# nabeelscicom/DistilCodec_nabeel

Measured on AMD Instinct MI355X. Metric: 24 kHz samples/s encode+decode at 1/8 GPU; code-index bit-exact vs CPU, higher is better.
Workload: dtype f32

## Files before the change

### distilcodec_nabeel_amd/csrc/dcx_conv_h3.hip

```cpp
#include "dcx_conv_common.h"
#include "dcx_conv_launch.h"
#include "dcx_conv_pingpong.h"
#include "dcx_w3_layout.h"

namespace dcx {

DCX_DIAG_FILE(h3)

typedef _Float16 f16x8 __attribute__((ext_vector_type(8)));

template <int BM, int BN>
__device__ __forceinline__ bool ragged_tile_done(const ConvParams& p, const ConvParams& pr, int wg, int b, int ph) {
  int q0, co0;
  tile_origin<BM, BN>(p, wg, q0, co0);
  if (!tile_dead(p, pr, b, q0)) return false;
  epilogue_dead<BM, BN, 512>(p, pr, q0, co0, b, ph);
  return true;
}

template <int BN, int HALO, bool RAG = false>
__device__ __forceinline__ void x3dq_tile(const ConvParams& p, const ConvParams& pr, const int wg, const int b, const int ph) {
  constexpr int BM = 32768 / BN, WN = BN / 64, WM = 8 / WN;
  constexpr int NA = HALO ? 2 : 3;
  constexpr int WR = BM / WM, WC = BN / WN, TM = WR / 16, TN = WC / 16;
  constexpr int AR = BM + HALO;
  constexpr int A_G = AR / 16, B_G = BN / 16;
  constexpr int A_PW = A_G / 4, B_PW = B_G / 4;
  constexpr int ABUF = AR * 128, BBUF = BN * 128;
  constexpr int LDS_B = NA * ABUF + 3 * BBUF;
  static_assert(WR == 64 && WC == 64 && A_G % 4 == 0 && B_G % 4 == 0 && AR % 64 == 0, "tile shape");
  static_assert(LDS_B <= 160 * 1024, "LDS");
  __shared__ __attribute__((aligned(16))) unsigned short lds[LDS_B / 2];

  if constexpr (RAG)
    if (ragged_tile_done<BM, BN>(p, pr, wg, b, ph)) return;
  const TileGeo g = tile_geo<BM, BN, WN>(p, wg, ph, p.Cin / 32);
  const int lane = g.lane, group = g.group, gw = g.gw, wm = g.wm, wn = g.wn, q0 = g.q0, co0 = g.co0;
  const int nchunks = g.nchunks, taps = g.taps, nsteps = g.nsteps, lo_rel = g.lo_rel, row0 = g.row0;
  const int arow = p.ldx * 4;
  const __amdgpu_buffer_rsrc_t rx = x_desc<4, HALO>(p, b, row0, BM);
  const int rbase = HALO ? row0 : 0;
  const __amdgpu_buffer_rsrc_t rw = __builtin_amdgcn_make_buffer_rsrc(
      (void*)(p.w3 + w3_step(taps, p.Cin, p.Cout, ph, 0, 0)), 0, taps * nchunks * p.Cout * 128, 0x00020000);

  int a_off[A_PW], b_off[B_PW];
#pragma unroll
  for (int i = 0; i < A_PW; ++i) {
    const int u = (group * A_G + i * 4 + gw) * 64;
    const int pc = u / AR, row = u - pc * AR + lane;
    a_off[i] = (rbase + row) * arow + (pc & 3) * 32 + (pc >> 2) * 16;
  }
#pragma unroll
  for (int i = 0; i < B_PW; ++i) {
    b_off[i] = w3_wide_lane(co0, lane) + w3_wide_piece(BN, group * B_G + i * 4 + gw);
  }
  unsigned short* const a_dst = lds + (group * A_G + gw) * 512;
  unsigned short* const b_dst = lds + NA * ABUF / 2 + (group * B_G + gw) * 512;
  [[maybe_unused]] bool in_loop = false;
  auto dma_step = [&](int c, int m, int slot) {
#ifdef DCX_X3_NODMA
    if (in_loop) return 0;
#endif
    int n = B_PW;
    if (m == 0) {
#pragma unroll
      for (int i = 0; i < A_PW; ++i)
        dma16(rx, a_dst + (HALO ? (c & 1) : slot) * (ABUF / 2) + i * 2048, a_off[i] + c * 128, 0);
      n += A_PW;
    }
    const int soff = w3_step_bytes(nchunks, p.Cout, m, c);
#pragma unroll
    for (int i = 0; i < B_PW; ++i) dma16(rw, b_dst + slot * (BBUF / 2) + i * 2048, b_off[i], soff);
    return n;
  };

  const int l15 = lane & 15, kg = lane >> 4;
  const int pah = kg * AR * 16, pal = (4 + kg) * AR * 16;
  const int pbh = kg * BN * 16, pbl = (4 + kg) * BN * 16;
  const char* const ldsb = reinterpret_cast<const char*>(lds);
  const int bcol = NA * ABUF + (wn * WC + l15) * 16;
  s16x8 aq[TM][2], bq[TN][2];
  auto readF = [&](int c, int m, int slot) {
    const char* a = ldsb + (HALO ? (c & 1) : slot) * ABUF + (wm * WR + m * p.in_step - lo_rel + l15) * 16;
    const char* bb = ldsb + bcol + slot * BBUF;
#pragma unroll
    for (int j = 0; j < TN; ++j) {
      bq[j][0] = *reinterpret_cast<const s16x8*>(bb + j * 256 + pbh);
      bq[j][1] = *reinterpret_cast<const s16x8*>(bb + j * 256 + pbl);
    }
#pragma unroll
    for (int i = 0; i < TM; ++i) {
      aq[i][0] = *reinterpret_cast<const s16x8*>(a + i * 256 + pah);
      aq[i][1] = *reinterpret_cast<const s16x8*>(a + i * 256 + pal);
    }
  };
  f32x4 acc[TM][TN];
  zero_acc(acc);
  auto mfma = [&]() {
    __builtin_amdgcn_s_setprio(1);
#pragma unroll
    for (int k = 0; k < 3; ++k) {
      const int sa = k == 1 ? 1 : 0, sb = k == 0 ? 1 : 0;
#pragma unroll
      for (int i = 0; i < TM; ++i)
#pragma unroll
        for (int j = 0; j < TN; ++j)
          acc[i][j] = __builtin_amdgcn_mfma_f32_16x16x32_f16(__builtin_bit_cast(f16x8, aq[i][sa]),
                                                             __builtin_bit_cast(f16x8, bq[j][sb]), acc[i][j], 0, 0, 0);
    }
    __builtin_amdgcn_s_setprio(0);
  };

  const StepPos l3 = pingpong3_prologue(nsteps, taps, dma_step);
  const EpiPre epre = epi_range_pre<HALO == 0 ? 3 : 0>(p, pr, b);
  const float unscale = __builtin_bit_cast(float, __builtin_amdgcn_readfirstlane(__builtin_bit_cast(int,
      __builtin_ldexpf(1.0f, -(p.w3_shift + (pr.x_ash ? pr.x_ash[b] : pr.x_ash_c))))));
  pingpong3_drain();
  in_loop = true;
  pingpong3_loop<true>(group, nsteps, taps, l3, dma_step, readF, mfma);
#pragma unroll
  for (int i = 0; i < TM; ++i)
#pragma unroll
    for (int j = 0; j < TN; ++j) acc[i][j] *= unscale;
  epilogue_lds<BM, BN, WM, WN, LDS_B / 4, 512, HALO == 0 ? 3 : 0, RAG>(p, pr, acc, q0, co0, b, ph, reinterpret_cast<float*>(lds), &epre);
}

template <int BN, int HALO, bool RAG = false>
__global__ void __launch_bounds__(512, 2) conv_gemm_x3dq(const ConvParams p) {
  int wg, b, ph;
  flat_tile(((p.Lq + 32768 / BN - 1) / (32768 / BN)) * (p.Cout / BN), p.batch, wg, b, ph);
  x3dq_tile<BN, HALO, RAG>(p, p, wg, b, ph);
}

template <int BN, bool RAG = false>
__global__ void __launch_bounds__(512, 2) conv_gemm_x3dq_group(const ConvGroup g) {
  ConvParams p;
  int local, b;
  const ConvParams& pr = group_member(g, p, local, b);
  x3dq_tile<BN, 64, RAG>(p, pr, local, b, 0);
}

template <int HALO, bool SPLIT, int BN = 256, bool RAG = false>
__device__ __forceinline__ void x3dw_tile(const ConvParams& p, const ConvParams& pr, const int wg, const int b, const int ph) {
  constexpr int BM = BN == 256 ? 256 : 384, WN = BN / 128, WM = 8 / WN;
  constexpr int WR = BM / WM, WC = 128, TM = WR / 16, TN = WC / 16;
  constexpr int AR = BM + HALO;
  constexpr int A_N = AR / 8, B_N = BN / 8;
  constexpr int A_PW = A_N / 4;
  constexpr int ABUF = AR * 128, BBUF = BN * 128;
  constexpr int NA = 2;
  constexpr int LDS_B = NA * ABUF + 2 * BBUF;
  static_assert(A_N % 4 == 0 && B_N % 4 == 0 && AR % 64 == 0, "tile shape");
  static_assert(LDS_B + 16 <= 160 * 1024, "LDS");
  __shared__ __attribute__((aligned(16))) unsigned short lds[LDS_B / 2 + 8];
  unsigned int* const rd_cnt = reinterpret_cast<unsigned int*>(lds + LDS_B / 2);

  const int tid = threadIdx.x, lane = tid & 63;
  [[maybe_unused]] const int wave = tid >> 6;
  const int group = __builtin_amdgcn_readfirstlane(tid >> 8);
  const int gw = __builtin_amdgcn_readfirstlane((tid >> 6) & 3);
  const int wm = wave / WN, wn = wave % WN;
  const int ntiles = p.Cout / BN;
  const int mt = wg / ntiles, nt = wg - mt * ntiles;
  const int q0 = mt * BM, co0 = nt * BN;
  if (RAG && tile_dead(p, pr, b, q0)) {
    epilogue_dead<BM, BN, 512>(p, pr, q0, co0, b, ph);
    return;
  }
  const int nchunks = p.Cin / 32;
  const int taps = p.taps;
  const int nsteps = nchunks * taps;
  const int lo_rel = p.in_step < 0 ? (taps - 1) * p.in_step : 0;
  const int row0 = q0 + p.in_base[ph] + lo_rel;
  const int arow = p.ldx * 4;
  const __amdgpu_buffer_rsrc_t rx = x_desc<4, HALO>(p, b, row0, BM);
  const int rbase = HALO ? row0 : 0;
  const __amdgpu_buffer_rsrc_t rw = __builtin_amdgcn_make_buffer_rsrc(
      (void*)(p.w3 + w3_step(taps, p.Cin, p.Cout, ph, 0, 0)), 0, taps * nchunks * p.Cout * 128, 0x00020000);

  const int a_lane = (rbase + lane) * arow;
  const int b_lane = w3_wide_lane(co0, lane);
  [[maybe_unused]] bool in_loop = false;
  auto dmaA1 = [&](int c, int slot, int i) {
#ifdef DCX_X3_NODMA
    if (in_loop) return;
#endif
    const int k = i * 4 + gw;
    const int u = k * 64, pc = u / AR, row = u - pc * AR;
    const int abuf = HALO ? (c & 1) : slot;
    dma16(rx, lds + abuf * (ABUF / 2) + k * 512, a_lane + row * arow + (pc & 3) * 32 + (pc >> 2) * 16 + c * 128, 0);
  };
#ifndef DCX_X3W_BG0_DIV
#define DCX_X3W_BG0_DIV 2
#endif
  constexpr int B_G0 = !SPLIT ? B_N : HALO ? B_N / DCX_X3W_BG0_DIV : 0;
  constexpr int B_W0 = B_G0 / 4, B_W1 = (B_N - B_G0) / 4;
  auto dmaB1 = [&](int c, int m, int slot, int i) {
#ifdef DCX_X3_NODMA
    if (in_loop) return;
#endif
    const int k = (group ? B_G0 : 0) + i * 4 + gw;
    dma16(rw, lds + NA * ABUF / 2 + slot * (BBUF / 2) + k * 512, b_lane, w3_step_bytes(nchunks, p.Cout, m, c) + w3_wide_piece(BN, k));
  };
  auto dma_step = [&](int c, int m, int slot) {
    if (m == 0) {
#pragma unroll
      for (int i = 0; i < A_PW; ++i) dmaA1(c, slot, i);
    }
#pragma unroll
    for (int i = 0; i < B_W0; ++i) dmaB1(c, m, slot, i);
  };
  auto dma_step1 = [&](int c, int m, int slot) {
#pragma unroll
    for (int i = 0; i < B_W1; ++i) dmaB1(c, m, slot, i);
  };

  const int l15 = lane & 15, kg = lane >> 4;
  const char* const ldsb = reinterpret_cast<const char*>(lds);
  const char* const a_rd = ldsb + kg * AR * 16 + (wm * WR + l15) * 16;
  const char* const b_rd = ldsb + NA * ABUF + kg * BN * 16 + (wn * WC + l15) * 16;
  s16x8 aq[TM][2], bq[TN][2];
  auto readF = [&](int c, int m, int slot) {
    const char* a = a_rd + ((HALO ? (c & 1) : slot) * ABUF + (m * p.in_step - lo_rel) * 16);
    const char* bb = b_rd + slot * BBUF;
#pragma unroll
    for (int j = 0; j < TN; ++j) {
      bq[j][0] = *reinterpret_cast<const s16x8*>(bb + j * 256);
      bq[j][1] = *reinterpret_cast<const s16x8*>(bb + j * 256 + 4 * BN * 16);
    }
#pragma unroll
    for (int i = 0; i < TM; ++i) {
      aq[i][0] = *reinterpret_cast<const s16x8*>(a + i * 256);
      aq[i][1] = *reinterpret_cast<const s16x8*>(a + i * 256 + 4 * AR * 16);
    }
  };
  f32x4 acc[TM][TN];
  zero_acc(acc);
  auto mfma = [&]() {
    __builtin_amdgcn_s_setprio(1);
#pragma unroll
    for (int k = 0; k < 3; ++k) {
      const int sa = k == 1 ? 1 : 0, sb = k == 0 ? 1 : 0;
#pragma unroll
      for (int i = 0; i < TM; ++i) {
#pragma unroll
        for (int j = 0; j < TN; ++j)
          acc[i][j] = __builtin_amdgcn_mfma_f32_16x16x32_f16(__builtin_bit_cast(f16x8, aq[i][sa]),
                                                             __builtin_bit_cast(f16x8, bq[j][sb]), acc[i][j], 0, 0, 0);
      }
    }
    __builtin_amdgcn_s_setprio(0);
  };

  int cl = 0, ml = 0;
  if (SPLIT && tid == 0) *rd_cnt = 0u;
  for (int t = 0; t < 2 && t < nsteps; ++t) {
    if (group == 0) dma_step(cl, ml, t);
    else if (SPLIT) dma_step1(cl, ml, t);
    step_adv(cl, ml, taps);
  }
  const EpiPre epre = epi_range_pre<HALO == 0 ? 3 : 0>(p, pr, b);
  const float unscale = __builtin_bit_cast(float, __builtin_amdgcn_readfirstlane(__builtin_bit_cast(int,
      __builtin_ldexpf(1.0f, -(p.w3_shift + (pr.x_ash ? pr.x_ash[b] : pr.x_ash_c))))));
  asm volatile("s_waitcnt vmcnt(0)" ::: "memory");
  seg_barrier();
  in_loop = true;
#ifdef DCX_SEG_DIAG
  unsigned long long sd[6] = {};
#endif
  int cr = 0, mr = 0;
  if (group == 0) {
    readF(0, 0, 0);
    if (SPLIT) {
      asm volatile("s_waitcnt lgkmcnt(0)" ::: "memory");
      if (lane == 0) __hip_atomic_fetch_add(rd_cnt, 1u, __ATOMIC_RELAXED, __HIP_MEMORY_SCOPE_WORKGROUP);
    }
    step_adv(cr, mr, taps);
    for (int s = 0; s < nsteps; ++s) {
      DCX_SEGT(ta);
      mfma();
      asm volatile("s_waitcnt vmcnt(0)" ::: "memory");
      DCX_SEGT(tb);
      seg_barrier();
      DCX_SEGT(tc);
      if (s + 2 < nsteps) {
        dma_step(cl, ml, s & 1);
        step_adv(cl, ml, taps);
      }
      DCX_SEGT(tr);
      if (s + 1 < nsteps) readF(cr, mr, (s + 1) & 1);
      DCX_SEGT(tq);
      DCX_SEGT(td);
      seg_barrier();
      DCX_SEGT(te);
#ifdef DCX_SEG_DIAG
      sd[0] += tb - ta; sd[1] += tc - tb; sd[2] += td - tc; sd[3] += te - td; sd[4] += tr - tc; sd[5] += tq - tr;
#endif
      step_adv(cr, mr, taps);
    }
  } else {
    for (int s = 0; s < nsteps; ++s) {
      DCX_SEGT(ta);
      readF(cr, mr, s & 1);
      if (SPLIT) {
        int n = 0;
        if (s + 2 < nsteps) {
          asm volatile("s_waitcnt lgkmcnt(0)" ::: "memory");
          if (lane == 0) __hip_atomic_fetch_add(rd_cnt, 1u, __ATOMIC_RELAXED, __HIP_MEMORY_SCOPE_WORKGROUP);
          const unsigned int want = 4u * (unsigned)(s + 2);
          while (__hip_atomic_load(rd_cnt, __ATOMIC_RELAXED, __HIP_MEMORY_SCOPE_WORKGROUP) < want) {
          }
          dma_step1(cl, ml, s & 1);
          step_adv(cl, ml, taps);
          n = B_W1;
        }
        wait_dma(n);
      }
      DCX_SEGT(tb);
      seg_barrier();
      DCX_SEGT(tc);
      mfma();
      DCX_SEGT(td);
      seg_barrier();
      DCX_SEGT(te);
#ifdef DCX_SEG_DIAG
      sd[2] += tb - ta; sd[3] += tc - tb; sd[0] += td - tc; sd[1] += te - td; sd[5] += tb - ta;
#endif
      step_adv(cr, mr, taps);
    }
  }
#ifdef DCX_SEG_DIAG
  if ((threadIdx.x & 255) == 0) {
#pragma unroll
    for (int i = 0; i < 6; ++i) atomicAdd(&g_seg_diag[group * 6 + i], sd[i]);
    if (group == 0) atomicAdd(&g_seg_diag[12], (unsigned long long)nsteps);
  }
  if (lane == 0) {
#pragma unroll
    for (int i = 0; i < 6; ++i) atomicAdd(&g_seg_diag8[wave * 6 + i], sd[i]);
    if (wave == 0) atomicAdd(&g_seg_diag8[48], (unsigned long long)nsteps);
  }
#endif
  asm volatile("s_waitcnt vmcnt(0)" ::: "memory");
#pragma unroll
  for (int i = 0; i < TM; ++i)
#pragma unroll
    for (int j = 0; j < TN; ++j) acc[i][j] *= unscale;
  epilogue_lds<BM, BN, WM, WN, LDS_B / 4, 512, HALO == 0 ? 3 : 0, RAG>(p, pr, acc, q0, co0, b, ph, reinterpret_cast<float*>(lds), &epre);
}

template <int HALO, bool SPLIT, int BN = 256, bool RAG = false>
__global__ void __launch_bounds__(512, 2) conv_gemm_x3dw(const ConvParams p) {
  constexpr int BM = BN == 256 ? 256 : 384;
  int wg, b, ph;
  flat_tile(((p.Lq + BM - 1) / BM) * (p.Cout / BN), p.batch, wg, b, ph);
  x3dw_tile<HALO, SPLIT, BN, RAG>(p, p, wg, b, ph);
}

template <bool SPLIT, int BN = 256, bool RAG = false>
__global__ void __launch_bounds__(512, 2) conv_gemm_x3dw_group(const ConvGroup g) {
  ConvParams p;
  int local, b;
  const ConvParams& pr = group_member(g, p, local, b);
  x3dw_tile<64, SPLIT, BN, RAG>(p, pr, local, b, 0);
}

bool x3dq_ok(const ConvParams& p, int bn, bool wide) {
  const int span = (p.taps - 1) * (p.in_step < 0 ? -p.in_step : p.in_step);
  if (!p.x6 || !p.w3 || p.x_layout != LAYOUT_H2 || p.Cin % 32 || p.Cout % bn || p.ksplit > 1) return false;
  const long long arow = (long long)p.ldx * 4;
  if ((long long)p.taps * p.Cin * p.Cout * 4 >= (1LL << 31)) return false;
  if (p.taps == 1) {
    for (int i = 0; i < kMaxPhases; ++i)
      if (p.in_base[i] < 0) return false;
    return 256LL * arow < (1LL << 31);
  }
  return p.taps >= (wide ? 2 : 3) && span > 0 && span <= 64 && (long long)(p.Lin + 1024) * arow < (1LL << 31);
}
int x3dq_bn(const ConvParams& p) {
  const int k = p.kn ? p.kn->h3_bn : 0;
  if (p.Cout % 256) return (k == 128 && p.taps >= 3) || p.taps < 2 ? 128 : 384;
  if (p.taps == 2) return 512;
  return k == 128 ? 128 : k == 256 ? 256 : 512;
}

template <int BN>
hipError_t launch_x3dq(const ConvParams& p, int batch, int phases, hipStream_t s, const char** kname) {
  constexpr int BM = 32768 / BN;
  if (p.taps == 1) {
    if (p.clip_len) return hipErrorNotSupported;
    if (kname) *kname = BN == 256 ? "conv_gemm_x3dm<128,256>" : "conv_gemm_x3dm<256,128>";
    return launch_flat<BM, BN>(conv_gemm_x3dq<BN, 0>, p, batch, phases, 512, s);
  }
  if (kname) *kname = BN == 256 ? "conv_gemm_x3dq<128,256,halo>" : "conv_gemm_x3dq<256,128,halo>";
  if (p.clip_len) return launch_flat<BM, BN>(conv_gemm_x3dq<BN, 64, true>, p, batch, phases, 512, s);
  return launch_flat<BM, BN>(conv_gemm_x3dq<BN, 64>, p, batch, phases, 512, s);
}

template hipError_t launch_x3dq<256>(const ConvParams&, int, int, hipStream_t, const char**);
template hipError_t launch_x3dq<128>(const ConvParams&, int, int, hipStream_t, const char**);

hipError_t launch_x3dw(const ConvParams& p, int bsel, int batch, int phases, hipStream_t s, const char** kname) {
  const bool sp = knobs(p).h3_split;
  if (p.clip_len) {
    if (p.taps == 1) return hipErrorNotSupported;
    if (bsel == 384) {
      if (kname) *kname = "conv_gemm_x3dw<384,128,halo>";
      return sp ? launch_flat<384, 128>(conv_gemm_x3dw<64, true, 128, true>, p, batch, phases, 512, s)
                : launch_flat<384, 128>(conv_gemm_x3dw<64, false, 128, true>, p, batch, phases, 512, s);
    }
    if (kname) *kname = "conv_gemm_x3dw<256,256,halo>";
    return sp ? launch_flat<256, 256>(conv_gemm_x3dw<64, true, 256, true>, p, batch, phases, 512, s)
              : launch_flat<256, 256>(conv_gemm_x3dw<64, false, 256, true>, p, batch, phases, 512, s);
  }
  if (bsel == 384) {
    if (kname) *kname = "conv_gemm_x3dw<384,128,halo>";
    return sp ? launch_flat<384, 128>(conv_gemm_x3dw<64, true, 128>, p, batch, phases, 512, s)
              : launch_flat<384, 128>(conv_gemm_x3dw<64, false, 128>, p, batch, phases, 512, s);
  }
  if (p.taps == 1) {
    if (kname) *kname = "conv_gemm_x3dw<256,256>";
    return sp ? launch_flat<256, 256>(conv_gemm_x3dw<0, true>, p, batch, phases, 512, s)
              : launch_flat<256, 256>(conv_gemm_x3dw<0, false>, p, batch, phases, 512, s);
  }
  if (kname) *kname = "conv_gemm_x3dw<256,256,halo>";
  return sp ? launch_flat<256, 256>(conv_gemm_x3dw<64, true>, p, batch, phases, 512, s)
            : launch_flat<256, 256>(conv_gemm_x3dw<64, false>, p, batch, phases, 512, s);
}

hipError_t launch_h3_group(const ConvGroup& g, int bsel, bool split, unsigned blocks, hipStream_t s, const char** kname) {
  if (g.p[0].clip_len) {
    if (bsel == 384) {
      if (kname) *kname = "conv_gemm_x3dw_group<384,128,halo>";
      if (split) hipLaunchKernelGGL((conv_gemm_x3dw_group<true, 128, true>), dim3(blocks), dim3(512), 0, s, g);
      else hipLaunchKernelGGL((conv_gemm_x3dw_group<false, 128, true>), dim3(blocks), dim3(512), 0, s, g);
    } else if (bsel == 512) {
      if (kname) *kname = "conv_gemm_x3dw_group<256,256,halo>";
      if (split) hipLaunchKernelGGL((conv_gemm_x3dw_group<true, 256, true>), dim3(blocks), dim3(512), 0, s, g);
      else hipLaunchKernelGGL((conv_gemm_x3dw_group<false, 256, true>), dim3(blocks), dim3(512), 0, s, g);
    } else if (bsel == 256) {
      if (kname) *kname = "conv_gemm_x3dq_group<128,256,halo>";
      hipLaunchKernelGGL((conv_gemm_x3dq_group<256, true>), dim3(blocks), dim3(512), 0, s, g);
    } else {
      if (kname) *kname = "conv_gemm_x3dq_group<256,128,halo>";
      hipLaunchKernelGGL((conv_gemm_x3dq_group<128, true>), dim3(blocks), dim3(512), 0, s, g);
    }
    return hipGetLastError();
  }
  if (bsel == 384) {
    if (kname) *kname = "conv_gemm_x3dw_group<384,128,halo>";
    if (split) hipLaunchKernelGGL((conv_gemm_x3dw_group<true, 128>), dim3(blocks), dim3(512), 0, s, g);
    else hipLaunchKernelGGL((conv_gemm_x3dw_group<false, 128>), dim3(blocks), dim3(512), 0, s, g);
  } else if (bsel == 512) {
    if (kname) *kname = "conv_gemm_x3dw_group<256,256,halo>";
    if (split) hipLaunchKernelGGL(conv_gemm_x3dw_group<true>, dim3(blocks), dim3(512), 0, s, g);
    else hipLaunchKernelGGL(conv_gemm_x3dw_group<false>, dim3(blocks), dim3(512), 0, s, g);
  } else if (bsel == 256) {
    if (kname) *kname = "conv_gemm_x3dq_group<128,256,halo>";
    hipLaunchKernelGGL((conv_gemm_x3dq_group<256>), dim3(blocks), dim3(512), 0, s, g);
  } else {
    if (kname) *kname = "conv_gemm_x3dq_group<256,128,halo>";
    hipLaunchKernelGGL((conv_gemm_x3dq_group<128>), dim3(blocks), dim3(512), 0, s, g);
  }
  return hipGetLastError();
}

}
```

Baseline: 49.09 million.

## Use row-blocked XOR-swizzled LDS layout for A tiles in x3dw kernel

Replaces the column-plane LDS layout of the activation tile in the x3dw conv GEMM with a row-major 8-row block layout where each 128-byte row holds all k-pieces, XOR-swizzled by row bits. The DMA lanes now load 8 rows by 8 pieces per instruction, and the fragment reads use an XOR on the address to pick the second half-plane, which removes the per-instruction divide and aims to cut LDS bank conflicts and improve global coalescing. The new layout applies to every variant except the plain halo, non-split, BN=256, non-ragged, non-grouped case, which keeps the old path. It relies on the swizzle staying conflict-free when the rows are shifted by the halo offset.

```diff
diff --git a/distilcodec_nabeel_amd/csrc/dcx_a3_layout.h b/distilcodec_nabeel_amd/csrc/dcx_a3_layout.h
--- /dev/null
+++ b/distilcodec_nabeel_amd/csrc/dcx_a3_layout.h
@@ -0,0 +1,25 @@
+#pragma once
+
+#if defined(__HIPCC__) || defined(__CUDACC__)
+#define DCX_A3_HD __host__ __device__
+#else
+#define DCX_A3_HD
+#endif
+
+namespace dcx {
+
+constexpr int kA3BlockRows = 8;
+constexpr int kA3PlaneXor = 64;
+
+DCX_A3_HD constexpr int a3_swz(int row, int q) { return q ^ (row & 6); }
+DCX_A3_HD constexpr int a3_image(int row, int q) { return row * 128 + a3_swz(row, q) * 16; }
+
+DCX_A3_HD constexpr int a3_lane_row(int lane) { return lane >> 3; }
+DCX_A3_HD constexpr int a3_lane_piece(int lane) { return a3_swz(lane >> 3, lane & 7); }
+DCX_A3_HD constexpr int a3_piece_src(int q) { return (q & 3) * 32 + (q >> 2) * 16; }
+DCX_A3_HD constexpr int a3_src_lane(int rbase, int arow, int lane) {
+  return (rbase + a3_lane_row(lane)) * arow + a3_piece_src(a3_lane_piece(lane));
+}
+DCX_A3_HD constexpr int a3_src_inst(int arow, int k, int c) { return k * kA3BlockRows * arow + c * 128; }
+
+}
diff --git a/distilcodec_nabeel_amd/csrc/dcx_conv_h3.hip b/distilcodec_nabeel_amd/csrc/dcx_conv_h3.hip
--- a/distilcodec_nabeel_amd/csrc/dcx_conv_h3.hip
+++ b/distilcodec_nabeel_amd/csrc/dcx_conv_h3.hip
@@ -1,6 +1,7 @@
 #include "dcx_conv_common.h"
 #include "dcx_conv_launch.h"
 #include "dcx_conv_pingpong.h"
+#include "dcx_a3_layout.h"
 #include "dcx_w3_layout.h"
 
 namespace dcx {
@@ -140,7 +141,7 @@
   x3dq_tile<BN, 64, RAG>(p, pr, local, b, 0);
 }
 
-template <int HALO, bool SPLIT, int BN = 256, bool RAG = false>
+template <int HALO, bool SPLIT, int BN = 256, bool RAG = false, bool GROUPED = false>
 __device__ __forceinline__ void x3dw_tile(const ConvParams& p, const ConvParams& pr, const int wg, const int b, const int ph) {
   constexpr int BM = BN == 256 ? 256 : 384, WN = BN / 128, WM = 8 / WN;
   constexpr int WR = BM / WM, WC = 128, TM = WR / 16, TN = WC / 16;
@@ -178,7 +179,8 @@
   const __amdgpu_buffer_rsrc_t rw = __builtin_amdgcn_make_buffer_rsrc(
       (void*)(p.w3 + w3_step(taps, p.Cin, p.Cout, ph, 0, 0)), 0, taps * nchunks * p.Cout * 128, 0x00020000);
 
-  const int a_lane = (rbase + lane) * arow;
+  constexpr bool ROWS = !(HALO && !SPLIT && BN == 256 && !RAG && !GROUPED);
+  const int a_lane = ROWS ? a3_src_lane(rbase, arow, lane) : (rbase + lane) * arow;
   const int b_lane = w3_wide_lane(co0, lane);
   [[maybe_unused]] bool in_loop = false;
   auto dmaA1 = [&](int c, int slot, int i) {
@@ -186,9 +188,13 @@
     if (in_loop) return;
 #endif
     const int k = i * 4 + gw;
-    const int u = k * 64, pc = u / AR, row = u - pc * AR;
     const int abuf = HALO ? (c & 1) : slot;
-    dma16(rx, lds + abuf * (ABUF / 2) + k * 512, a_lane + row * arow + (pc & 3) * 32 + (pc >> 2) * 16 + c * 128, 0);
+    if constexpr (ROWS) {
+      dma16(rx, lds + abuf * (ABUF / 2) + k * 512, a_lane + a3_src_inst(arow, k, c), 0);
+    } else {
+      const int u = k * 64, pc = u / AR, row = u - pc * AR;
+      dma16(rx, lds + abuf * (ABUF / 2) + k * 512, a_lane + row * arow + (pc & 3) * 32 + (pc >> 2) * 16 + c * 128, 0);
+    }
   };
 #ifndef DCX_X3W_BG0_DIV
 #define DCX_X3W_BG0_DIV 2
@@ -217,11 +223,15 @@
 
   const int l15 = lane & 15, kg = lane >> 4;
   const char* const ldsb = reinterpret_cast<const char*>(lds);
-  const char* const a_rd = ldsb + kg * AR * 16 + (wm * WR + l15) * 16;
+  const int a_row = wm * WR + l15;
+  static_assert(WR % kA3BlockRows == 0 && a3_image(16, 0) == 2048, "row blocks as immediates");
   const char* const b_rd = ldsb + NA * ABUF + kg * BN * 16 + (wn * WC + l15) * 16;
   s16x8 aq[TM][2], bq[TN][2];
   auto readF = [&](int c, int m, int slot) {
-    const char* a = a_rd + ((HALO ? (c & 1) : slot) * ABUF + (m * p.in_step - lo_rel) * 16);
+    const int a_r = a_row + (HALO ? m * p.in_step - lo_rel : 0);
+    const int ah = (HALO ? (c & 1) : slot) * ABUF + (ROWS ? a3_image(a_r, kg) : kg * AR * 16 + a_r * 16);
+    const char* a = ldsb + ah;
+    const char* al = ldsb + (ROWS ? ah ^ kA3PlaneXor : ah + 4 * AR * 16);
     const char* bb = b_rd + slot * BBUF;
 #pragma unroll
     for (int j = 0; j < TN; ++j) {
@@ -230,8 +240,8 @@
     }
 #pragma unroll
     for (int i = 0; i < TM; ++i) {
-      aq[i][0] = *reinterpret_cast<const s16x8*>(a + i * 256);
-      aq[i][1] = *reinterpret_cast<const s16x8*>(a + i * 256 + 4 * AR * 16);
+      aq[i][0] = *reinterpret_cast<const s16x8*>(a + i * (ROWS ? 2048 : 256));
+      aq[i][1] = *reinterpret_cast<const s16x8*>(al + i * (ROWS ? 2048 : 256));
     }
   };
   f32x4 acc[TM][TN];
@@ -362,7 +372,7 @@
   ConvParams p;
   int local, b;
   const ConvParams& pr = group_member(g, p, local, b);
-  x3dw_tile<64, SPLIT, BN, RAG>(p, pr, local, b, 0);
+  x3dw_tile<64, SPLIT, BN, RAG, true>(p, pr, local, b, 0);
 }
 
 bool x3dq_ok(const ConvParams& p, int bn, bool wide) {
```

Result: faster. 51.53 million (median of 6 runs) (+5.0%).
